# manyeyes/K2TransducerAsr

Measured on AMD Instinct MI355X. Metric: RTFx (audio-sec/wall-sec) offline Zipformer greedy, higher is better.
Workload: dtype f32

## Files before the change

include/k2hip_debug.h:

```cpp
#ifndef K2HIP_DEBUG_H
#define K2HIP_DEBUG_H
#include "k2hip.h"

#ifdef __cplusplus
extern "C" {
#endif
#if defined(__GNUC__)
#pragma GCC visibility push(default)
#endif


int32_t k2hip_debug_search_retries(k2hip_model_t* model, int32_t* n);
int32_t k2hip_debug_decoder_table_check(k2hip_model_t* model, int32_t n_samples, uint32_t seed, int64_t* rows, int64_t* mismatched);
int32_t k2hip_debug_beam_trace(k2hip_model_t* model, int32_t* trace, int64_t cap_words, int32_t* B, int32_t* Tprime, int32_t* beam);

int32_t k2hip_debug_stream_hotword_uploads(k2hip_model_t* model, int32_t* uploads, int32_t* resident);
int32_t k2hip_debug_beam_launch_counts(int64_t* plain, int64_t* hotwords);

int32_t k2hip_debug_poison_stream(k2hip_online_stream_t* s);
int32_t k2hip_debug_stream_mirrored(const k2hip_online_stream_t* s, int32_t* ok);

int32_t k2hip_debug_gemm_run(k2hip_model_t* model, const float* A, const float* W, const float* bias, const float* res, float* C,
                             int32_t M, int32_t N, int32_t K, int32_t act, int32_t glu, int32_t glu_cols, int32_t cfg);
int32_t k2hip_debug_op_run(k2hip_model_t* model, const char* op, const int64_t* iargs, int32_t n_iargs, void* const* bufs,
                           const int64_t* buf_bytes, int32_t n_bufs, uint32_t out_mask);

int32_t k2hip_debug_kws_stream_get_state(const k2hip_kws_stream_t* s, float* a, int32_t* start, int32_t cap);
int32_t k2hip_debug_keywords_get_tables(const k2hip_keywords_t* kw, int32_t* parent, int32_t* tok, int32_t* depth, int32_t* keyword, float* bar,
                                        int32_t cap);
int32_t k2hip_debug_kws_ref_dp(const int32_t* parent, const int32_t* depth, const int32_t* keyword, const float* bar, int32_t S, const float* stay,
                               const float* emit, int32_t T, float* a, int32_t* start, int32_t* ev_keyword, int32_t* ev_start, int32_t* ev_end,
                               float* ev_sum, int32_t cap, int32_t* n_events);

int32_t k2hip_debug_ctc_kws_stream_get_state(const k2hip_ctc_kws_stream_t* s, float* v, int32_t* st, int32_t cap);
int32_t k2hip_debug_ctc_kws_ref_dp(const int32_t* parent, const int32_t* tok, const int32_t* depth, const int32_t* keyword, const float* bar,
                                   const int32_t* rc, int32_t S, const float* log_probs, int32_t V, int32_t T, float* v, int32_t* st,
                                   int32_t* ev_keyword, int32_t* ev_start, int32_t* ev_end, float* ev_sum, int32_t cap, int32_t* n_events);

int32_t k2hip_debug_gemm(k2hip_model_t* model, int32_t M, int32_t N, int32_t K, int32_t act, int32_t with_res, int32_t cfg,
                         int32_t iters, float* ms);
int32_t k2hip_debug_gemm_check(k2hip_model_t* model, int32_t M, int32_t N, int32_t K, int32_t act, int32_t with_res, int32_t cfg,
                               int32_t iters, float* ms, float* max_err);
int32_t k2hip_debug_gemm_trace(k2hip_model_t* model, int32_t M, int32_t N, int32_t K, int32_t act, int32_t with_res, int32_t cfg,
                               unsigned long long* out, int64_t cap, int32_t* n_wg, int32_t* n_waves);

#if defined(__GNUC__)
#pragma GCC visibility pop
#endif
#ifdef __cplusplus
}
#endif
#endif
```

k2transducerasr_amd/csrc/api.cpp:

```cpp
#include <algorithm>
#include <atomic>
#include <cmath>
#include <fstream>
#include <iterator>
#include <map>
#include <memory>
#include <mutex>
#include <new>

#include "text.h"
#include "engine.h"
#include "beam_hist.h"
#include "ctc_prefix_hist.h"
#include "hotwords.h"
#include "keywords.h"
#include "kws_ref.h"
#include "ctc_kws_ref.h"
#include "ngram_lm.h"
#include "../../include/k2hip_debug.h"

using namespace k2hip;

struct PinVec {
    Engine* e = nullptr;
// ... 2484 lines not shown
int32_t k2hip_debug_decoder_table_check(k2hip_model_t* model, int32_t n_samples, uint32_t seed,
                                                                                int64_t* rows, int64_t* mismatched) {
    return guard([&] {
        NEED(model); NEED(rows); NEED(mismatched);
        K2_REQUIRE(n_samples >= 0 && n_samples <= 65536, "decoder table check: %d samples", n_samples);
        EngineLock lk(model->engine);
        long long r = 0, m = 0;
        model->engine.decoder_table_check(n_samples, seed, &r, &m);
        *rows = r;
        *mismatched = m;
    });
}
int32_t k2hip_debug_poison_stream(k2hip_online_stream_t* s) {
    return guard([&] {
        NEED(s);
        s->poisoned = true;
    });
}

int32_t k2hip_debug_stream_mirrored(const k2hip_online_stream_t* s, int32_t* ok) {
    return guard([&] {
        NEED(s); NEED(ok);
        *ok = s->mir_ok ? 1 : 0;
    });
}

int32_t k2hip_debug_set_switch(const char* env_name, int32_t value) {
    return guard([&] {
        NEED(env_name);
        tunables_init_from_env();
        if (!tunables_set(env_name, value)) failf(K2HIP_ERR_INVALID, "unknown switch '%s'", env_name);
    });
}
int32_t k2hip_debug_gemm(k2hip_model_t* model, int32_t M, int32_t N, int32_t K,
                                                                 int32_t act, int32_t with_res, int32_t cfg, int32_t iters, float* ms) {
    return guard([&] {
        NEED(model); NEED(ms);
        EngineLock lk(model->engine);
        *ms = model->engine.debug_gemm(M, N, K, act, with_res != 0, iters, cfg, nullptr);
    });
}
int32_t k2hip_debug_gemm_check(k2hip_model_t* model, int32_t M, int32_t N, int32_t K,
                                                                       int32_t act, int32_t with_res, int32_t cfg, int32_t iters, float* ms,
                                                                       float* max_err) {
    return guard([&] {
        NEED(model); NEED(ms); NEED(max_err);
        EngineLock lk(model->engine);
        *ms = model->engine.debug_gemm(M, N, K, act, with_res != 0, iters, cfg, max_err);
    });
}

int32_t k2hip_debug_gemm_run(k2hip_model_t* model, const float* A, const float* W, const float* bias, const float* res, float* C, int32_t M,
                             int32_t N, int32_t K, int32_t act, int32_t glu, int32_t glu_cols, int32_t cfg) {
    return guard([&] {
        NEED(model); NEED(A); NEED(W); NEED(C);
        EngineLock lk(model->engine);
        model->engine.debug_gemm_host(A, W, bias, res, C, M, N, K, act, glu, glu_cols, cfg);
    });
}

int32_t k2hip_debug_op_run(k2hip_model_t* model, const char* op, const int64_t* iargs, int32_t n_iargs, void* const* bufs,
                           const int64_t* buf_bytes, int32_t n_bufs, uint32_t out_mask) {
    return guard([&] {
        NEED(model); NEED(op);
        if (!Engine::debug_op) failf(K2HIP_ERR_UNSUPPORTED, "debug_op_run: this build has no kernels");
        EngineLock lk(model->engine);
// ... 245 lines not shown
```

k2transducerasr_amd/csrc/engine.cpp:

```cpp
#include <cstring>
#include <thread>

#include "engine.h"
#include "lattice_ref.h"
#include "ctc_lattice_ref.h"
#include "kws_ref.h"
#include "ctc_kws_ref.h"
#include "ctc_prefix_bias_ref.h"
#include "ctc_prefix_ref.h"
#include "hotwords.h"
#include "ngram_lm.h"

#include <climits>
#include <cmath>

namespace k2hip {

namespace {
constexpr int kTailFrames = 19;
}

Engine::Engine(const std::string& weights, const char* overrides, int device) : device_(device) {
    tunables_init_from_env();
    model_.reset(new Model(weights, overrides));
// ... 381 lines not shown
            std::swap(src, src_alt);
            return;
        }
        linear(c, src, D, wi, bi, hid, HV, M, D, HV);
        if (site) {
            attn_av_out_ring(c, aw, ring(k == 1 ? lay_.val1[gl] : lay_.val2[gl]), hid, wo, bo, src, B, T, KL, KLp, H, vh, D);
            return;
        }
        if (attn_av_out(c, aw, hid, wo, bo, src, B, T, T, KLp, H, vh, D)) return;
        GemmArgs g;
        g.A = aw; g.lda = KLp; g.sA0 = (long long)T * KLp; g.sA1 = (long long)B * T * KLp;
        g.W = hid; g.w_kn = 1; g.ldw = HV; g.sW0 = (long long)T * HV; g.sW1 = vh;
        g.C = tmp; g.ldc = HV; g.sC0 = (long long)T * HV; g.sC1 = vh;
        g.M = T; g.N = vh; g.K = T; g.nb0 = B; g.nb1 = H;
        gemm(c, g);
        linear(c, tmp, HV, wo, bo, src, D, M, HV, D, ACT_NONE, src, D);
    };
    auto conv_module = [&](int k) {
        if (site) {
            const long long cache_off = k == 1 ? lay_.conv1[gl] : lay_.conv2[gl];
            const float *wc = wk("conv_module%d.depthwise_conv.causal_conv.weight", k), *bc = wk("conv_module%d.depthwise_conv.causal_conv.bias", k);
            const float *ww = wk("conv_module%d.depthwise_conv.chunkwise_conv.weight", k), *bw = wk("conv_module%d.depthwise_conv.chunkwise_conv.bias", k);
            const float* sc = wk("conv_module%d.depthwise_conv.chunkwise_conv_scale", k);
            bool fused = false;
            if (!tunables().no_fused_conv)
                fused = gemm_glu_causal_conv(c, src, wk("conv_module%d.in_proj.weight#glu", k), wk("conv_module%d.in_proj.bias#glu", k), online_pool_, SS,
                                             cache_off, site->d_slots, wc, bc, ww, bw, sc, tmp2, B, T, D, K);
            if (!fused) {
                linear(c, src, D, wk("conv_module%d.in_proj.weight", k), wk("conv_module%d.in_proj.bias", k), hid, 2 * D, M, D, 2 * D);
                glu_causal_conv(c, hid, online_pool_, SS, cache_off, site->d_slots, wc, bc, ww, bw, sc, tmp2, B, T, D, K);
            }
        } else {
            const float *wd = wk("conv_module%d.depthwise_conv.weight#kd", k), *bd = wk("conv_module%d.depthwise_conv.bias", k);
            if (M >= 256 && !tunables().no_glu_epilogue) {
                GemmArgs g;
                g.A = src; g.lda = D; g.W = wk("conv_module%d.in_proj.weight#glu", k); g.ldw = D; g.bias = wk("conv_module%d.in_proj.bias#glu", k);
                g.C = hid; g.ldc = D; g.M = M; g.N = 2 * D; g.K = D; g.glu = 1;
                gemm(c, g);
                dwconv1d_swoosh(c, hid, wd, bd, tmp2, B, T, D, K);
            } else {
                linear(c, src, D, wk("conv_module%d.in_proj.weight", k), wk("conv_module%d.in_proj.bias", k), hid, 2 * D, M, D, 2 * D);
                glu_dwconv1d_swoosh(c, hid, wd, bd, tmp2, B, T, D, K);
            }
        }
        linear(c, tmp2, D, wk("conv_module%d.out_proj.weight", k), wk("conv_module%d.out_proj.bias", k), src, D, M, D, D, ACT_NONE, src, D);
    };

    linear(c, cat, ldcat, w("feed_forward1.out_proj.weight"), w("feed_forward1.out_proj.bias"), src, D, M, F1, D, ACT_NONE, x, D);
    nonlin_attention();
    self_attn(1);
    conv_module(1);
    {
        linear(c, src, D, w("feed_forward2.in_proj.weight"), w("feed_forward2.in_proj.bias"), hid, F, M, D, F, ACT_SWOOSH_L);
        GemmArgs g;
        g.A = hid; g.lda = F; g.W = w("feed_forward2.out_proj.weight"); g.ldw = F; g.bias = w("feed_forward2.out_proj.bias");
        g.C = src; g.ldc = D; g.M = M; g.N = D; g.K = F; g.res = src; g.ldr = D;
        g.byp_orig = x; g.ld_orig = D; g.byp_scale = w("bypass_mid.bypass_scale");
        gemm(c, g);
    }
    self_attn(2);
    conv_module(2);
    feed_forward(3, F * 5 / 4, src, src);
    if (tail && tail->bias2)
        biasnorm_bypass_downsample(c, src, x, w("norm.bias"), w("norm.log_scale"), w("bypass.bypass_scale"), x, tail->bias2, tail->xd2, B, T, D,
                                   tail->ds2, tail->D2);
    else
        biasnorm_bypass(c, src, x, w("norm.bias"), w("norm.log_scale"), w("bypass.bypass_scale"), x, M, D);
// ... 1781 lines not shown
            g.glu = I(); g.glu_cols = I();
            g.ldm = I(); g.sM0 = L(); g.sM1 = L();
            g.ld_orig = I();
            const int cfg = I(), res_is_C = I();
            const long long oA = L(), oW = L(), oR = L(), oC = L(), oM = L(), oO = L();
            float *A = P(), *W = P(), *bias = P(), *res = P(), *C = P();
            const int* skip = reinterpret_cast<const int*>(P());
            float *mul = P(), *orig = P(), *scale = P();
            int* plan_out = reinterpret_cast<int*>(P());
            K2_REQUIRE(A && W && C && plan_out && buf_bytes[n_bufs - 1] >= 20, "debug_op_run gemm: A, W, C and a plan buffer of 5 ints are needed");
            K2_REQUIRE(!(res_is_C && res), "debug_op_run gemm: res_is_C takes no res buffer");
            K2_REQUIRE(oA >= 0 && oW >= 0 && oR >= 0 && oC >= 0 && oM >= 0 && oO >= 0, "debug_op_run gemm: negative offset");
            if (res_is_C) res = C;
            g.A = A + oA; g.W = W + oW; g.bias = bias; g.res = res ? res + oR : nullptr; g.C = C + oC;
            g.skip_if_zero = skip;
            g.mul = mul ? mul + oM : nullptr;
            g.byp_orig = orig ? orig + oO : nullptr; g.byp_scale = scale;
            GemmForceGuard force(cfg);
            const GemmPlan pl = plan_gemm(g, gemm_force());
            const int rep[5] = {(int)pl.family, pl.idx, pl.BM, pl.BN, pl.mode};
            K2_HIP(copy_blocking(plan_out, rep, sizeof rep, hipMemcpyHostToDevice));
            gemm(c, g);
        } else if (name == "gemm_glu_causal_conv") {
            float *x = P(), *wg = P(), *bg = P(), *pool = P();
            const long long ss = L(), off = L();
            const int* slots = reinterpret_cast<const int*>(P());
            float *wc = P(), *bc = P(), *ww = P(), *bw = P(), *sc = P(), *y = P();
            const int B = I(), Tc = I(), D = I(), K = I();
            int* entry_out = reinterpret_cast<int*>(P());
            K2_REQUIRE(entry_out && buf_bytes[n_bufs - 1] >= 4, "debug_op_run gemm_glu_causal_conv: an entry buffer of 1 int is needed");
            const int entry = glu_conv_ring_entry(B, Tc, D, K);
            K2_HIP(copy_blocking(entry_out, &entry, sizeof entry, hipMemcpyHostToDevice));
            took = gemm_glu_causal_conv(c, x, wg, bg, pool, ss, off, slots, wc, bc, ww, bw, sc, y, B, Tc, D, K);
        } else if (name == "biasnorm") {
            float *x = P(), *bias = P(), *ls = P(), *y = P();
            const int M = I(), D = I();
            biasnorm(c, x, bias, ls, y, M, D);
        } else if (name == "bypass") {
            float *orig = P(), *x = P(), *scale = P(), *y = P();
            const int M = I(), D = I();
            bypass(c, orig, x, scale, y, M, D);
        } else if (name == "biasnorm_bypass") {
            float *x = P(), *orig = P(), *nb = P(), *ls = P(), *scale = P(), *y = P();
            const int M = I(), D = I();
            biasnorm_bypass(c, x, orig, nb, ls, scale, y, M, D);
        } else if (name == "biasnorm_bypass_downsample") {
            float *x = P(), *orig = P(), *nb = P(), *ls = P(), *scale = P(), *y = P(), *bias2 = P(), *xd2 = P();
            const int B = I(), T = I(), D = I(), ds2 = I(), D2 = I();
            biasnorm_bypass_downsample(c, x, orig, nb, ls, scale, y, bias2, xd2, B, T, D, ds2, D2);
        } else if (name == "downsample") {
            float *x = P(), *bias = P(), *y = P();
            const int B = I(), T = I(), D = I(), ds = I(), Din = I();
            downsample(c, x, bias, y, B, T, D, ds, Din);
        } else if (name == "downsample_full") {
            FullDimSegs s;
            s.n = I();
            K2_REQUIRE(s.n >= 1 && s.n <= 8, "debug_op_run downsample_full: %d segments", s.n);
            for (int k = 0; k < s.n; k++) s.ld[k] = I();
            for (int k = 0; k < s.n; k++) s.col1[k] = I();
            s.lz_Td = I(); s.lz_ds = I(); s.lz_Do = I();
            for (int k = 0; k < s.n; k++) s.src[k] = P();
            s.lz_orig = P(); s.lz_xd = P(); s.lz_scale = P();
            float *bias = P(), *y = P();
            const int B = I(), T = I(), D = I(), ds = I();
            downsample_full(c, s, bias, y, B, T, D, ds);
        } else if (name == "upsample_combine") {
// ... 764 lines not shown
```

k2transducerasr_amd/csrc/gemm.hip:

```cpp
#include <algorithm>
#include <cmath>
#include <cstdlib>
#include <map>
#include <mutex>
#include <type_traits>

#include "act.h"
#include "kernels.h"

#pragma clang diagnostic ignored "-Winline-asm"

namespace k2hip {

typedef float f32x16 __attribute__((ext_vector_type(16)));
typedef float f32x4 __attribute__((ext_vector_type(4)));

namespace {


__device__ __forceinline__ float apply_act(float v, int act) {
    switch (act) {
        case ACT_SWOOSH_L: return swoosh_l(v);
        case ACT_SWOOSH_R: return swoosh_r(v);
        case ACT_TANH: {
// ... 471 lines not shown
                if (e == 0 && gk < 3) {
                    __builtin_amdgcn_sched_barrier(0);
#pragma unroll
                    for (int i = 0; i < MT; i++)
                        fa[nx][i] = *reinterpret_cast<const float4*>(sa + i * 32 * BK + (((2 * (gk + 1) + lh) ^ swa) << 2));
#pragma unroll
                    for (int j = 0; j < NT; j++)
                        fb[nx][j] = *reinterpret_cast<const float4*>(sb + j * 32 * BK + (((2 * (gk + 1) + lh) ^ swb) << 2));
                    __builtin_amdgcn_sched_barrier(0);
                }
            }
        }
    }

    K2_DMA_STAMP()
#pragma unroll
    for (int j = 0; j < NT; j++)
#pragma unroll
        for (int i = 0; i < MT; i++) {
            float vals[16];
#pragma unroll
            for (int r = 0; r < 16; r++) vals[r] = acc[i][j][r];
            epilogue_rows<16, Rows32>(g, vals, m0 + wr * WM + i * 32 + 4 * lh, n0 + wc * WN + j * 32 + li, C, nullptr, rres[i][j], R != nullptr,
                                      nullptr, g.bias ? g.bias + z0 * g.sBias0 : nullptr);
        }
    K2_DMA_STAMP()
    if (stamp && lane == 0) {
        stamp[62] = nstamp;
        stamp[63] = __builtin_amdgcn_s_memrealtime();
    }
#undef K2_DMA_STAMP
}

template <int BM, int BN, int WM, int WN, int NST>
__global__ __launch_bounds__(64 * (BM / WM) * (BN / WN)) void gemm_f32_mfma_pipe(GemmArgs g) {
    constexpr int BK = 32;
    constexpr int MT = WM / 32, NT = WN / 32;
    constexpr int WCOLS = BN / WN;
    constexpr int NW = (BM / WM) * (BN / WN);
    constexpr int NINST = (BM + BN) / 8;
    constexpr int IPW = NINST / NW;
    constexpr int STAGE = (BM + BN) * BK;
    constexpr int DPE = (IPW + 3) / 4;
    static_assert(NST == 3 || NST == 4, "pipe: three or four stages");
    static_assert(NINST % NW == 0, "pipe: every wave issues the same number of DMA instructions");
    static_assert((NST - 2) * IPW <= 63 && MT <= 4 && NT <= 2, "pipe: counted wait / wave tile out of range");

    if (g.skip_if_zero && *g.skip_if_zero == 0) return;
    extern __shared__ __attribute__((aligned(16))) float smem[];

    const int tid = threadIdx.x;
    const int lane = tid & 63, wave = __builtin_amdgcn_readfirstlane(tid >> 6);
    const int wr = wave / WCOLS, wc = wave % WCOLS;
    const int li = lane & 31, lh = lane >> 5;
    float* __restrict__ C = g.C;
    const float* __restrict__ R = g.res;
    int mb_, nb_;
    xcd_tile(mb_, nb_, g.xcd_panels == 1 ? 0 : g.M, g.N);
    const int m0 = mb_ * BM, n0 = nb_ * BN;
    const int nk = g.K / BK;

    unsigned long long* stamp = g.dbg ? g.dbg + ((size_t)(blockIdx.x + blockIdx.y * gridDim.x) * NW + wave) * 64 : nullptr;
    int nstamp = 0;
#define K2_PIPE_STAMP()                                                    \
    if (stamp) {  \
        if (lane == 0) stamp[nstamp] = __builtin_amdgcn_s_memtime();       \
        nstamp++;                                                          \
    }
    if (stamp && lane == 0) stamp[60] = __builtin_amdgcn_s_memrealtime();
    K2_PIPE_STAMP()

    const unsigned lds_base = (unsigned)(unsigned long long)(__attribute__((address_space(3))) char*)smem;
    unsigned voff[IPW];
    unsigned long long sb[IPW];
    unsigned mq[IPW];
#pragma unroll
    for (int q = 0; q < IPW; q++) {
        const int inst = wave + q * NW;
        const int slot = inst * 64 + lane;
        const int r = slot >> 3, cp = slot & 7;
        const int c = cp ^ ((r >> 1) & 7);
        const bool is_a = inst < BM / 8;
        const long long row = is_a ? min(m0 + r, g.M - 1) : min(n0 + (r - BM), g.N - 1);
        voff[q] = (unsigned)((row * (is_a ? g.lda : g.ldw) + 4 * c) * 4);
        const unsigned long long base = (unsigned long long)(is_a ? g.A : g.W);
        sb[q] = ((unsigned long long)(unsigned)__builtin_amdgcn_readfirstlane((int)(base >> 32)) << 32) |
                (unsigned long long)(unsigned)__builtin_amdgcn_readfirstlane((int)(unsigned)base);
        mq[q] = __builtin_amdgcn_readfirstlane(lds_base + inst * 1024);
    }

#define K2_PIPE_DMA(ST_, KT_, q_)                                                                                          \
    {                                                                                                                      \
// ... 66 lines not shown
        }

    f32x16 acc[MT][NT];
#pragma unroll
    for (int i = 0; i < MT; i++)
#pragma unroll
        for (int j = 0; j < NT; j++)
#pragma unroll
            for (int r = 0; r < 16; r++) acc[i][j][r] = 0.f;
    f32x4 fa[2][MT], fb[2][NT];
    K2_PIPE_STAMP()
    if (nk >= NST - 1) asm volatile("s_waitcnt vmcnt(%0)" ::"n"((NST - 2) * IPW) : "memory");
    else asm volatile("s_waitcnt vmcnt(0)" ::: "memory");
    __builtin_amdgcn_s_barrier();
    K2_PIPE_READ(0, 0, 0)
    K2_PIPE_STAMP()
    float rres[MT][NT][16];
    if (R) {
#pragma unroll
        for (int j = 0; j < NT; j++) {
            const int col = min(n0 + wc * WN + j * 32 + li, g.N - 1);
#pragma unroll
            for (int i = 0; i < MT; i++)
#pragma unroll
                for (int r = 0; r < 16; r++) {
                    const int row = min(m0 + wr * WM + i * 32 + (r & 3) + 8 * (r >> 2) + 4 * lh, g.M - 1);
                    rres[i][j][r] = R[(long long)row * g.ldr + col];
                }
        }
    }
    float bias_pre[NT];
#pragma unroll
    for (int j = 0; j < NT; j++) bias_pre[j] = g.bias ? g.bias[min(n0 + wc * WN + j * 32 + li, g.N - 1)] : 0.f;

    int kt = 0;
    const int nsteady = nk - (NST - 1);
    for (; kt + NST <= nsteady; kt += NST) {
        K2_PIPE_STEP(0, kt, true, true, K2_PIPE_WAIT_STEADY)
        K2_PIPE_STEP(1, kt + 1, true, true, K2_PIPE_WAIT_STEADY)
        K2_PIPE_STEP(2, kt + 2, true, true, K2_PIPE_WAIT_STEADY)
        if (NST == 4) { K2_PIPE_STEP(NST == 4 ? 3 : 0, kt + 3, true, true, K2_PIPE_WAIT_STEADY) }
    }
#define K2_PIPE_S(j_) K2_PIPE_STEP((j_) % NST, kt + (j_), true, true, K2_PIPE_WAIT_STEADY)
#define K2_PIPE_T(j_) K2_PIPE_STEP((j_) % NST, kt + (j_), true, false, K2_PIPE_WAIT_DRAIN)
#define K2_PIPE_L(j_) K2_PIPE_STEP((j_) % NST, kt + (j_), false, false, K2_PIPE_WAIT_DRAIN)
    const int rs = nsteady - kt;
    if (NST == 3) {
        switch (rs) {
            case 0: K2_PIPE_T(0) K2_PIPE_L(1) break;
            case 1: K2_PIPE_S(0) K2_PIPE_T(1) K2_PIPE_L(2) break;
            default: K2_PIPE_S(0) K2_PIPE_S(1) K2_PIPE_T(2) K2_PIPE_L(3) break;
        }
    } else {
        switch (rs) {
            case 0: K2_PIPE_T(0) K2_PIPE_T(1) K2_PIPE_L(2) break;
            case 1: K2_PIPE_S(0) K2_PIPE_T(1) K2_PIPE_T(2) K2_PIPE_L(3) break;
            case 2: K2_PIPE_S(0) K2_PIPE_S(1) K2_PIPE_T(2) K2_PIPE_T(3) K2_PIPE_L(4) break;
            default: K2_PIPE_S(0) K2_PIPE_S(1) K2_PIPE_S(2) K2_PIPE_T(3) K2_PIPE_T(4) K2_PIPE_L(5) break;
        }
    }
#undef K2_PIPE_S
#undef K2_PIPE_T
#undef K2_PIPE_L
    K2_PIPE_STAMP()
#undef K2_PIPE_WAIT_DRAIN
#undef K2_PIPE_WAIT_STEADY
#undef K2_PIPE_STEP
#undef K2_PIPE_FRAGS_READY
#undef K2_PIPE_READ
#undef K2_PIPE_DMA

#pragma unroll
    for (int j = 0; j < NT; j++)
#pragma unroll
        for (int i = 0; i < MT; i++) {
            float vals[16];
#pragma unroll
            for (int r = 0; r < 16; r++) vals[r] = acc[i][j][r];
            epilogue_rows<16, Rows32>(g, vals, m0 + wr * WM + i * 32 + 4 * lh, n0 + wc * WN + j * 32 + li, C, nullptr, rres[i][j], R != nullptr,
                                      nullptr, g.bias, true, bias_pre[j]);
        }
    K2_PIPE_STAMP()
    if (stamp && lane == 0) {
        stamp[62] = nstamp;
        stamp[63] = __builtin_amdgcn_s_memrealtime();
    }
#undef K2_PIPE_STAMP
}

template <int BM, int BN, int WM, int WN, int NST>
__global__ __launch_bounds__(64 * (BM / WM) * (BN / WN)) void gemm_f32_mfma_p16(GemmArgs g) {
    constexpr int BK = 32;
    constexpr int MT = WM / 16, NT = WN / 16;
    constexpr int WCOLS = BN / WN;
    constexpr int NW = (BM / WM) * (BN / WN);
    constexpr int NINST = (BM + BN) / 8;
    constexpr int IPW = NINST / NW;
    constexpr int STAGE = (BM + BN) * BK;
    constexpr int DPE = (IPW + 3) / 4;
    static_assert(NST == 3, "p16: three stages");
    static_assert(NINST % NW == 0, "p16: every wave issues the same number of DMA instructions");
    static_assert(MT >= 1 && NT >= 1 && MT * NT <= 12, "p16: wave tile");

    if (g.skip_if_zero && *g.skip_if_zero == 0) return;
// ... 644 lines not shown
    lds_attr.ensure(gemm_f32_mfma_dma<BM, BN, WM, WN, NST>, (int)lds);
    hipLaunchKernelGGL((gemm_f32_mfma_dma<BM, BN, WM, WN, NST>), grid, dim3(64 * (BM / WM) * (BN / WN)), lds, ctx.stream, a);
}

template <int BM, int BN, int KS, int NST, int LW, int PF = 0>
void launch_ring(const Ctx& ctx, const GemmArgs& a) {
    dim3 grid(cdiv(a.N, BN), cdiv(a.M, BM), a.nb0 * a.nb1);
    size_t lds = sizeof(float) * std::max((size_t)NST * KS * (BM + BN) * 32, KS > 1 ? (size_t)KS * (BM / 32) * (BN / 32) * 1024 : (size_t)0) + (PF ? 256 : 0);
    static LdsAttrOnce lds_attr;
    lds_attr.ensure(gemm_f32_mfma_ring<BM, BN, KS, NST, LW, PF>, (int)lds);
    hipLaunchKernelGGL((gemm_f32_mfma_ring<BM, BN, KS, NST, LW, PF>), grid, dim3(64 * ((BM / 32) * (BN / 32) * KS + LW + PF)), lds, ctx.stream, a);
}

template <int BM, int BN, int KS, int NST, int PF = 0>
void launch_ring_conv(const Ctx& ctx, const GemmArgs& a) {
    dim3 grid(cdiv(a.N, BN), cdiv(a.M, BM), 1);
    const int pad = a.cf_K >> 1, Kc = (a.cf_K + 1) >> 1, CH = BN / 2;
    const size_t conv_fl = (size_t)(BM / a.cf_Tc) * CH * (pad + a.cf_Tc) + (size_t)CH * (Kc | 1) + (size_t)CH * a.cf_K;
    size_t lds = sizeof(float) * std::max({(size_t)NST * KS * (BM + BN) * 32, KS > 1 ? (size_t)KS * (BM / 32) * (BN / 32) * 1024 : (size_t)0, conv_fl}) + (PF ? 256 : 0);
    static LdsAttrOnce lds_attr;
    lds_attr.ensure(gemm_f32_mfma_ring<BM, BN, KS, NST, 0, PF, true>, (int)lds);
    hipLaunchKernelGGL((gemm_f32_mfma_ring<BM, BN, KS, NST, 0, PF, true>), grid, dim3(64 * ((BM / 32) * (BN / 32) * KS + PF)), lds, ctx.stream, a);
}

template <int BM, int BN, int WM, int WN, int NST>
void launch_pipe(const Ctx& ctx, const GemmArgs& a) {
    dim3 grid(cdiv(a.N, BN), cdiv(a.M, BM), 1);
    size_t lds = sizeof(float) * NST * (BM + BN) * 32;
    static LdsAttrOnce lds_attr;
    lds_attr.ensure(gemm_f32_mfma_pipe<BM, BN, WM, WN, NST>, (int)lds);
    K2_REQUIRE((long long)a.M * a.lda < (1ll << 29) && (long long)a.N * a.ldw < (1ll << 29), "pipe: operand too large for 31-bit lane byte offsets");
    K2_REQUIRE(a.K % 32 == 0 && a.K >= 32 * (NST - 1), "pipe: K %d too short for %d stages", a.K, NST);
    hipLaunchKernelGGL((gemm_f32_mfma_pipe<BM, BN, WM, WN, NST>), grid, dim3(64 * (BM / WM) * (BN / WN)), lds, ctx.stream, a);
}

template <int BM, int BN, int WM, int WN, int NST>
void launch_p16(const Ctx& ctx, const GemmArgs& a) {
    dim3 grid(cdiv(a.N, BN), cdiv(a.M, BM), 1);
    size_t lds = sizeof(float) * NST * (BM + BN) * 32;
    static LdsAttrOnce lds_attr;
    lds_attr.ensure(gemm_f32_mfma_p16<BM, BN, WM, WN, NST>, (int)lds);
    K2_REQUIRE((long long)a.M * a.lda < (1ll << 29) && (long long)a.N * a.ldw < (1ll << 29), "p16: operand too large for 31-bit lane byte offsets");
    K2_REQUIRE(a.K % 32 == 0 && a.K >= 32 * (NST - 1) && !a.glu, "p16: K %d too short for %d stages, or a gated epilogue", a.K, NST);
    hipLaunchKernelGGL((gemm_f32_mfma_p16<BM, BN, WM, WN, NST>), grid, dim3(64 * (BM / WM) * (BN / WN)), lds, ctx.stream, a);
}

template <int BM, int BN, int WM, int WN, int BK, int MODE>
void launch_cfg(const Ctx& ctx, const GemmArgs& a) {
    constexpr int LDSK = BK + 4;
    dim3 grid(cdiv(a.N, BN), cdiv(a.M, BM), a.nb0 * a.nb1);
    size_t lds = sizeof(float) * 2 * (BM + BN) * LDSK;
    static LdsAttrOnce lds_attr;
    lds_attr.ensure(gemm_f32_mfma<BM, BN, WM, WN, BK, MODE>, (int)lds);
    hipLaunchKernelGGL((gemm_f32_mfma<BM, BN, WM, WN, BK, MODE>), grid, dim3(64 * (BM / WM) * (BN / WN)), lds, ctx.stream, a);
}

template <int MODE>
void launch_reg(const Ctx& ctx, const GemmArgs& a, int idx) {
    switch (idx) {
#define X(i, bm, bn, wm, wn, bk) case i: launch_cfg<bm, bn, wm, wn, bk, MODE>(ctx, a); break;
        K2_REG_TABLE(X)
#undef X
    }
}

template <int E>
// ... 72 lines not shown
    K2_HIP(hipGetLastError());
    if (ctx.instrument && ctx.gemm_log)
        ctx.gemm_log->push_back({a.M, a.N, a.K, a.nb0 * a.nb1, a.act, a.res != nullptr, gemm_kind(a, p), 0.f});
    if (ctx.instrument) K2_HIP(hipEventRecord(ctx.next_event(), ctx.stream));
}

bool gemm_glu_causal_conv(const Ctx& ctx, const float* x, const float* wg, const float* bg, float* pool, long long slot_stride, long long off,
                          const int* slots, const float* wc, const float* bc, const float* ww, const float* bw, const float* sc, float* y, int B,
                          int Tc, int D, int K) {
    const int M = B * Tc, N = 2 * D;
    const int entry = glu_conv_ring_entry(B, Tc, D, K);
    if (entry < 0) return false;
    const double fl = 2.0 * M * (double)N * D;
    ctx.add_flops(fl, 2.0 * M * (double)D * (K + (K + 1) / 2), 1);
    if (ctx.dry) return true;
    GemmArgs g;
    g.A = x; g.lda = D; g.W = wg; g.ldw = D; g.bias = bg; g.C = y; g.ldc = D; g.M = M; g.N = N; g.K = D;
    g.cf_pool = pool; g.cf_stride = slot_stride; g.cf_off = off; g.cf_slots = slots;
    g.cf_wc = wc; g.cf_bc = bc; g.cf_ww = ww; g.cf_bw = bw; g.cf_sc = sc; g.cf_Tc = Tc; g.cf_K = K;
    g.xcd_panels = tunables().xcd_panels;
    if (ctx.instrument) K2_HIP(hipEventRecord(ctx.next_event(), ctx.stream));
    if (ctx.instrument && ctx.gemm_log) ctx.gemm_log->push_back({M, N, D, 1, 0, 0, 64, 0.f});
    switch (entry) {
        case 16: launch_ring_conv_entry<16>(ctx, g); break;
        case 17: launch_ring_conv_entry<17>(ctx, g); break;
        case 12: launch_ring_conv_entry<12>(ctx, g); break;
        default: launch_ring_conv_entry<8>(ctx, g); break;
    }
    K2_HIP(hipGetLastError());
    if (ctx.instrument) K2_HIP(hipEventRecord(ctx.next_event(), ctx.stream));
    return true;
}

void linear(const Ctx& ctx, const float* A, int lda, const float* W, const float* bias, float* C, int ldc, int M, int K,
            int N, int act, const float* res, int ldr) {
    GemmArgs g;
    g.A = A; g.lda = lda; g.W = W; g.ldw = K; g.bias = bias; g.C = C; g.ldc = ldc;
    g.M = M; g.N = N; g.K = K; g.act = act; g.res = res; g.ldr = ldr;
    gemm(ctx, g);
}

}
```

k2transducerasr_amd/csrc/gemm_plan.cpp:

```cpp
#include "kernels.h"

namespace k2hip {

namespace {

GemmForce g_force;

bool entry(GemmFamily f, int idx, GemmPlan* p) {
    p->family = f;
    p->idx = idx;
    switch (f) {
#define X(i, bm, bn, wm, wn, bk_or_nst) case i: p->BM = bm; p->BN = bn; p->waves = (bm / wm) * (bn / wn); return true;
        case GemmFamily::REG: switch (idx) { K2_REG_TABLE(X) } return false;
        case GemmFamily::DMA: switch (idx) { K2_DMA_TABLE(X) } return false;
        case GemmFamily::PIPE: switch (idx) { K2_PIPE_TABLE(X) } return false;
        case GemmFamily::P16: switch (idx) { K2_P16_TABLE(X) } return false;
#undef X
        case GemmFamily::RING: {
            if (idx < 0 || idx >= (int)(sizeof(kRing) / sizeof(kRing[0]))) return false;
            const RingCfg& r = kRing[idx];
            p->BM = r.BM;
            p->BN = r.BN;
            p->waves = (r.BM / 32) * (r.BN / 32) * r.KS + r.LW + r.PF;
            return true;
// ... 130 lines not shown
            if (tiles >= 128 && cost < best_cost) return make(GemmFamily::P16, 0, f.ablate);
        }
        return make(GemmFamily::PIPE, best, f.ablate);
    }
    if (dma_ok && (cfg == 5 || cfg == 0 || (cfg >= 7 && cfg <= 11))) return make(GemmFamily::DMA, cfg == 7 ? 5 : cfg, f.ablate);
    GemmPlan r = make(GemmFamily::REG, cfg == 7 || cfg == 8 || cfg == 11 ? 5 : (cfg <= 5 || cfg == 12) ? cfg : 2, f.ablate);
    r.mode = a.cv_Fout > 0 ? MODE_CONV : a.w_kn ? MODE_WKN : MODE_PLAIN;
    return r;
}

int gemm_kind(const GemmArgs& a, const GemmPlan& p) {
    const int base = a.cv_Fout > 0 ? 1 : (a.w_kn ? 2 : 0);
    switch (p.family) {
        case GemmFamily::REG: return base;
        case GemmFamily::DMA: return base + 16;
        case GemmFamily::SKINNY3: case GemmFamily::SKINNY6: case GemmFamily::SKINNY6_8: return base + 32;
        case GemmFamily::RING: return base + 64;
        case GemmFamily::PIPE: return base + 128 + 256 * (p.BM / 32) + 4096 * (p.BN / 32);
        case GemmFamily::P16: return base + 128 + 256 * (p.BM / 32) + 4096 * (p.BN / 32) + (1 << 20);
    }
    return base;
}

int glu_conv_ring_entry(int B, int Tc, int D, int K) {
    const int M = B * Tc, N = 2 * D;
    if (Tc < 2 || 32 % Tc != 0 || D % 64 != 0 || (K != 31 && K != 15 && K != 7)) return -1;
    int e = small_ring_entry(M, N, D);
    if (e < 0) e = 8;
    const RingCfg& r = kRing[e];
    if ((long long)(r.BM / Tc) * (r.BN / 2) * (K >> 1) > 8ll * (r.BM / 32) * (r.BN / 32) * r.KS * 64) return -1;
    return e;
}

}
```

k2transducerasr_amd/csrc/kernels.h:

```cpp
#pragma once
#include "ctc_prefix_layout.h"
#include "common.h"

namespace k2hip {

#ifdef K2HIP_DEV
#define K2HIP_DEV_SWITCH(name, def) int name = def
#else
#define K2HIP_DEV_SWITCH(name, def) static constexpr int name = def
#endif
struct Tunables {
    int no_glu_epilogue = 0;
    int attn_long = 0;
    int no_fused_av = 0;
    int fused_vproj_min_t = 4;
    int no_fused_vproj = 0;
    int no_fused_conv = 0;
    int conformer_gemm_scores = 0;
    int dw7_tiled = 0;
    int dw1d_tt = 0;
    int lstm_seq = 0;
    int greedy_one_part = 0;
    int greedy_parts = 0;
    int beam_launches = 0;
// ... 63 lines not shown
    const float* W = nullptr;
    const float* bias = nullptr;
    const float* res = nullptr;
    float* C = nullptr;
    int M = 0, N = 0, K = 0;
    int lda = 0, ldw = 0, ldc = 0, ldr = 0;
    int act = ACT_NONE;
    int xcd_panels = 0;
    int act_cols = 0;
    int w_kn = 0;
    int nb0 = 1, nb1 = 1;
    const int* skip_if_zero = nullptr;
    long long sA0 = 0, sA1 = 0, sW0 = 0, sW1 = 0, sC0 = 0, sC1 = 0, sR0 = 0, sR1 = 0;
    long long sBias0 = 0;
    int cv_Fout = 0, cv_Tout = 0, cv_Tin = 0, cv_Fin = 0, cv_C = 0, cv_st = 1, cv_sf = 1;
    int seg_len = 0, seg_stride = 0;
    int res_div = 1;
    int act_after_res = 0;
    int glu = 0;
    int glu_cols = 0;
    const float* mul = nullptr;
    int ldm = 0;
    long long sM0 = 0, sM1 = 0;
    const float* byp_orig = nullptr;
    const float* byp_scale = nullptr;
    int ld_orig = 0;
    float* cf_pool = nullptr;
    long long cf_stride = 0, cf_off = 0;
    const int* cf_slots = nullptr;
    const float *cf_wc = nullptr, *cf_bc = nullptr, *cf_ww = nullptr, *cf_bw = nullptr, *cf_sc = nullptr;
    int cf_Tc = 0, cf_K = 0;
    unsigned long long* dbg = nullptr;
    int ablate = 0;
};
void gemm(const Ctx& ctx, const GemmArgs& a);
bool gemm_glu_causal_conv(const Ctx& ctx, const float* x, const float* wg, const float* bg, float* pool, long long slot_stride, long long off,
                          const int* slots, const float* wc, const float* bc, const float* ww, const float* bw, const float* sc, float* y, int B,
                          int Tc, int D, int K);

#define K2_PIPE_TABLE(X)                                                                                                       \
    X(0, 128, 64, 64, 32, 3) X(1, 128, 64, 32, 32, 3) X(2, 128, 128, 64, 64, 3) X(3, 128, 128, 64, 32, 3) X(4, 128, 64, 64, 32, 4)  \
    X(5, 64, 64, 32, 32, 3) X(6, 128, 128, 64, 64, 4) X(7, 64, 128, 32, 64, 3) X(8, 128, 128, 32, 32, 3) X(9, 128, 64, 32, 32, 4) \
    X(10, 64, 64, 64, 32, 3) X(11, 64, 64, 32, 64, 3) X(12, 256, 64, 64, 32, 3) X(13, 128, 32, 32, 32, 3) X(14, 128, 32, 64, 32, 3)
#define K2_P16_TABLE(X) X(0, 64, 96, 32, 48, 3) X(1, 128, 96, 64, 48, 3) X(2, 64, 192, 32, 96, 3) X(3, 32, 96, 16, 48, 3)
#define K2_RING_TABLE(X)                                                                                        \
    X(0, 128, 64, 1, 2, 0, 0) X(1, 128, 64, 1, 3, 0, 0) X(2, 128, 64, 1, 2, 0, 1) X(3, 128, 64, 1, 3, 0, 1) X(4, 128, 64, 1, 4, 0, 1)   \
    X(5, 64, 64, 1, 3, 0, 0) X(6, 64, 64, 1, 3, 0, 1) X(7, 64, 64, 1, 4, 0, 1) X(8, 64, 64, 2, 3, 0, 0) X(9, 64, 64, 2, 3, 0, 1)      \
    X(10, 64, 64, 4, 2, 0, 0) X(11, 64, 64, 4, 2, 0, 1) X(12, 32, 64, 2, 3, 0, 0) X(13, 32, 64, 4, 3, 0, 0) X(14, 32, 64, 4, 3, 0, 1)  \
    X(15, 32, 32, 4, 3, 0, 0) X(16, 32, 32, 4, 4, 0, 1) X(17, 64, 32, 4, 3, 0, 0) X(18, 128, 128, 1, 2, 0, 0) X(19, 128, 128, 1, 2, 0, 1) \
    X(20, 64, 128, 1, 3, 0, 0) X(21, 64, 128, 1, 3, 0, 1) X(22, 64, 96, 1, 3, 0, 0) X(23, 64, 96, 1, 3, 0, 1) X(24, 128, 96, 1, 2, 0, 1) \
    X(25, 128, 64, 1, 3, 2, 0) X(26, 128, 64, 1, 3, 2, 1) X(27, 128, 64, 2, 2, 0, 1) X(28, 64, 96, 2, 3, 0, 0) X(29, 64, 96, 2, 2, 0, 0) \
    X(30, 64, 96, 2, 2, 0, 1) X(31, 128, 96, 1, 3, 0, 0) X(32, 128, 96, 1, 3, 0, 1)
struct RingCfg { int BM, BN, KS, NST, LW, PF; };
#define X(i, bm, bn, ks, nst, lw, pf) {bm, bn, ks, nst, lw, pf},
constexpr RingCfg kRing[] = {K2_RING_TABLE(X)};
#undef X
#define K2_DMA_TABLE(X)                                                                                                          \
    X(0, 128, 128, 64, 32, 3) X(5, 128, 64, 32, 32, 2) X(8, 128, 64, 32, 32, 4) X(9, 64, 64, 32, 32, 2) X(10, 64, 64, 32, 32, 3) \
    X(11, 64, 96, 32, 32, 2) X(20, 32, 32, 32, 32, 4) X(21, 32, 64, 32, 32, 4)
#define K2_REG_TABLE(X)                                                                                                           \
    X(0, 128, 128, 64, 32, 32) X(1, 128, 128, 64, 32, 64) X(2, 64, 64, 32, 32, 32) X(3, 64, 64, 32, 32, 64) X(4, 128, 64, 32, 32, 64) \
    X(5, 128, 64, 32, 32, 32) X(12, 128, 32, 32, 32, 32)
enum GemmMode { MODE_PLAIN = 0, MODE_CONV = 1, MODE_WKN = 2 };

enum class GemmFamily { REG, DMA, PIPE, P16, RING, SKINNY3, SKINNY6, SKINNY6_8 };
struct GemmPlan {
    GemmFamily family = GemmFamily::REG;
    int idx = 0;
    int mode = MODE_PLAIN;
    int ablate = 0;
    int BM = 0, BN = 0, waves = 0;
};
struct GemmForce {
    enum Kind { AUTO, CFG, RING, PIPE, P16 } kind = AUTO;
    int idx = -1;
    int ablate = 0;
    bool dma = true;
};
GemmForce decode_gemm_force(int code);
GemmPlan plan_gemm(const GemmArgs& a, const GemmForce& f);
int gemm_kind(const GemmArgs& a, const GemmPlan& p);
int glu_conv_ring_entry(int B, int Tc, int D, int K);
void debug_force_gemm_cfg(int code);
GemmForce gemm_force();
struct GemmForceGuard {
    explicit GemmForceGuard(int code) { debug_force_gemm_cfg(code); }
    ~GemmForceGuard() { debug_force_gemm_cfg(-1); }
    GemmForceGuard(const GemmForceGuard&) = delete;
    GemmForceGuard& operator=(const GemmForceGuard&) = delete;
};
void linear(const Ctx& ctx, const float* A, int lda, const float* W, const float* bias, float* C, int ldc, int M, int K,
            int N, int act = ACT_NONE, const float* res = nullptr, int ldr = 0);

struct RingRef {
    float* pool = nullptr;
    long long slot_stride = 0;
    long long off = 0;
    const int* slots = nullptr;
    const int* chunks = nullptr;
};

void attn_scores_softmax(const Ctx& ctx, const float* qkp, int ld, const float* pp, float* aw, int B, int T, int Tp, int H, int qh = 32,
                         int koff0 = -1, int poff0 = -1);

bool attn_av_out(const Ctx& ctx, const float* aw, const float* v, const float* wout, const float* bias, float* x, int B, int T, int KL, int Tp,
                 int H, int vh, int D);
bool attn_av_out_ring(const Ctx& ctx, const float* aw, const RingRef& vals, const float* newrows, const float* wout, const float* bias, float* x,
                      int B, int T, int KL, int Tp, int H, int vh, int D);
void attn_proj_av_out_ring(const Ctx& ctx, const float* aw, const RingRef& vals, const float* xin, const float* win, const float* bin,
                           const float* wout, const float* bias, float* xout, int B, int T, int KL, int Tp, int H, int vh, int D);

void nonlin_av_out_ring(const Ctx& ctx, const float* aw, const RingRef& cache, const float* hid, int ldh, const float* wout, const float* bias,
                        float* x, int B, int T, int KL, int Tp, int Hc, int D);

void pad_logfloor(const Ctx& ctx, const float* packed, const long long* d_off, const long long* d_len, float* out, int B,
// ... 437 lines not shown
```

Before: 23890.

## Fuse offline conv-module GLU GEMM with depthwise conv and SwooshR epilogue

For the offline (non-streaming) Zipformer conv module, the pipe MFMA GEMM gains a templated epilogue. It applies bias and GLU, stages the gated rows of a whole stream in LDS with zero padding, runs the depthwise 1D conv (K=15 or 31) and SwooshR, then writes the final output. This removes the intermediate hidden tensor's global write and read and a separate conv kernel launch. It only applies when a whole stream fits in one row tile (T <= BM), and the planner rejects cases where one-tile-per-stream would add waves. Otherwise it falls back to the old path.

New measurement: 24170, median of 6. 1.2% higher.

```diff
diff --git a/include/k2hip_debug.h b/include/k2hip_debug.h
--- a/include/k2hip_debug.h
+++ b/include/k2hip_debug.h
@@ -22,6 +22,7 @@
 
 int32_t k2hip_debug_gemm_run(k2hip_model_t* model, const float* A, const float* W, const float* bias, const float* res, float* C,
                              int32_t M, int32_t N, int32_t K, int32_t act, int32_t glu, int32_t glu_cols, int32_t cfg);
+int32_t k2hip_debug_conv_fused_plan(int32_t B, int32_t T, int32_t D, int32_t K, int32_t streaming, int32_t* entry);
 int32_t k2hip_debug_op_run(k2hip_model_t* model, const char* op, const int64_t* iargs, int32_t n_iargs, void* const* bufs,
                            const int64_t* buf_bytes, int32_t n_bufs, uint32_t out_mask);
 
diff --git a/k2transducerasr_amd/csrc/api.cpp b/k2transducerasr_amd/csrc/api.cpp
--- a/k2transducerasr_amd/csrc/api.cpp
+++ b/k2transducerasr_amd/csrc/api.cpp
@@ -2540,6 +2540,13 @@
         if (!tunables_set(env_name, value)) failf(K2HIP_ERR_INVALID, "unknown switch '%s'", env_name);
     });
 }
+int32_t k2hip_debug_conv_fused_plan(int32_t B, int32_t T, int32_t D, int32_t K, int32_t streaming, int32_t* entry) {
+    return guard([&] {
+        NEED(entry);
+        tunables_init_from_env();
+        *entry = glu_dwconv_pipe_entry(B, T, D, K, streaming != 0);
+    });
+}
 int32_t k2hip_debug_gemm(k2hip_model_t* model, int32_t M, int32_t N, int32_t K,
                                                                  int32_t act, int32_t with_res, int32_t cfg, int32_t iters, float* ms) {
     return guard([&] {
diff --git a/k2transducerasr_amd/csrc/engine.cpp b/k2transducerasr_amd/csrc/engine.cpp
--- a/k2transducerasr_amd/csrc/engine.cpp
+++ b/k2transducerasr_amd/csrc/engine.cpp
@@ -437,7 +437,9 @@
             }
         } else {
             const float *wd = wk("conv_module%d.depthwise_conv.weight#kd", k), *bd = wk("conv_module%d.depthwise_conv.bias", k);
-            if (M >= 256 && !tunables().no_glu_epilogue) {
+            const bool fused = gemm_glu_dwconv1d(c, src, wk("conv_module%d.in_proj.weight#glu", k), wk("conv_module%d.in_proj.bias#glu", k), wd, bd, tmp2, B, T, D, K);
+            if (fused) {
+            } else if (M >= 256 && !tunables().no_glu_epilogue) {
                 GemmArgs g;
                 g.A = src; g.lda = D; g.W = wk("conv_module%d.in_proj.weight#glu", k); g.ldw = D; g.bias = wk("conv_module%d.in_proj.bias#glu", k);
                 g.C = hid; g.ldc = D; g.M = M; g.N = 2 * D; g.K = D; g.glu = 1;
@@ -2285,6 +2287,47 @@
             const int entry = glu_conv_ring_entry(B, Tc, D, K);
             K2_HIP(copy_blocking(entry_out, &entry, sizeof entry, hipMemcpyHostToDevice));
             took = gemm_glu_causal_conv(c, x, wg, bg, pool, ss, off, slots, wc, bc, ww, bw, sc, y, B, Tc, D, K);
+        } else if (name == "gemm_glu_dwconv1d") {
+            const int wg_k = nbuf + 1, bg_k = nbuf + 2;
+            float *x = P(), *wg = P(), *bg = P(), *wd = P(), *bd = P(), *y = P();
+            const int B = I(), T = I(), D = I(), K = I();
+            int* entry_out = reinterpret_cast<int*>(P());
+            K2_REQUIRE(x && wg && bg && wd && bd && y && entry_out && buf_bytes[n_bufs - 1] >= 4, "debug_op_run gemm_glu_dwconv1d: six operands and an entry buffer of 1 int are needed");
+            K2_REQUIRE(B >= 1 && T >= 1 && D >= 16 && D % 16 == 0 && K >= 1, "debug_op_run gemm_glu_dwconv1d: B %d T %d D %d K %d", B, T, D, K);
+            const int M = B * T;
+            const int entry = glu_dwconv_pipe_entry(B, T, D, K, false);
+            K2_HIP(copy_blocking(entry_out, &entry, sizeof entry, hipMemcpyHostToDevice));
+            auto scratch = [&](size_t floats) {
+                char* p = nullptr;
+                K2_HIP(hipMalloc(&p, floats * sizeof(float)));
+                d.base.push_back(p);
+                return reinterpret_cast<float*>(p);
+            };
+            const bool fused = gemm_glu_dwconv1d(c, x, wg, bg, wd, bd, y, B, T, D, K);
+            if (fused) {
+            } else if (M >= 256 && !tunables().no_glu_epilogue) {
+                float* hid = scratch((size_t)M * D);
+                GemmArgs g;
+                g.A = x; g.lda = D; g.W = wg; g.ldw = D; g.bias = bg;
+                g.C = hid; g.ldc = D; g.M = M; g.N = 2 * D; g.K = D; g.glu = 1;
+                gemm(c, g);
+                dwconv1d_swoosh(c, hid, wd, bd, y, B, T, D, K);
+            } else {
+                const float *hw = static_cast<const float*>(bufs[wg_k]), *hb = static_cast<const float*>(bufs[bg_k]);
+                std::vector<float> vw((size_t)2 * D * D), vb((size_t)2 * D);
+                for (int ch = 0; ch < D; ch++) {
+                    const int rv = 32 * (ch / 16) + ch % 16, rg = rv + 16;
+                    memcpy(&vw[(size_t)ch * D], &hw[(size_t)rv * D], sizeof(float) * D);
+                    memcpy(&vw[(size_t)(D + ch) * D], &hw[(size_t)rg * D], sizeof(float) * D);
+                    vb[ch] = hb[rv];
+                    vb[D + ch] = hb[rg];
+                }
+                float *wp = scratch(vw.size()), *bp = scratch(vb.size()), *hid = scratch((size_t)M * 2 * D);
+                K2_HIP(copy_blocking(wp, vw.data(), vw.size() * sizeof(float), hipMemcpyHostToDevice));
+                K2_HIP(copy_blocking(bp, vb.data(), vb.size() * sizeof(float), hipMemcpyHostToDevice));
+                linear(c, x, D, wp, bp, hid, 2 * D, M, D, 2 * D);
+                glu_dwconv1d_swoosh(c, hid, wd, bd, y, B, T, D, K);
+            }
         } else if (name == "biasnorm") {
             float *x = P(), *bias = P(), *ls = P(), *y = P();
             const int M = I(), D = I();
diff --git a/k2transducerasr_amd/csrc/gemm.hip b/k2transducerasr_amd/csrc/gemm.hip
--- a/k2transducerasr_amd/csrc/gemm.hip
+++ b/k2transducerasr_amd/csrc/gemm.hip
@@ -527,7 +527,7 @@
 #undef K2_DMA_STAMP
 }
 
-template <int BM, int BN, int WM, int WN, int NST>
+template <int BM, int BN, int WM, int WN, int NST, int DWK = 0>
 __global__ __launch_bounds__(64 * (BM / WM) * (BN / WN)) void gemm_f32_mfma_pipe(GemmArgs g) {
     constexpr int BK = 32;
     constexpr int MT = WM / 32, NT = WN / 32;
@@ -552,7 +552,7 @@
     const float* __restrict__ R = g.res;
     int mb_, nb_;
     xcd_tile(mb_, nb_, g.xcd_panels == 1 ? 0 : g.M, g.N);
-    const int m0 = mb_ * BM, n0 = nb_ * BN;
+    const int m0 = DWK > 0 ? mb_ * g.dw_T : mb_ * BM, n0 = nb_ * BN;
     const int nk = g.K / BK;
 
     unsigned long long* stamp = g.dbg ? g.dbg + ((size_t)(blockIdx.x + blockIdx.y * gridDim.x) * NW + wave) * 64 : nullptr;
@@ -685,6 +685,15 @@
     float bias_pre[NT];
 #pragma unroll
     for (int j = 0; j < NT; j++) bias_pre[j] = g.bias ? g.bias[min(n0 + wc * WN + j * 32 + li, g.N - 1)] : 0.f;
+    constexpr int DW_CH = BN / 2, DW_TT = DWK > 0 ? BM * DW_CH / (64 * NW) : 1;
+    static_assert(DWK == 0 || (DW_TT == 8 && DWK % 2 == 1 && (BM + DWK - 1) * DW_CH <= NST * STAGE), "pipe: conv tail's tile form");
+    float dw_tap[DWK > 0 ? DWK : 1], dw_bias = 0.f;
+    if constexpr (DWK > 0) {
+        const float* wp = g.dw_w + (n0 >> 1) + (tid & (DW_CH - 1));
+        dw_bias = g.dw_b[(n0 >> 1) + (tid & (DW_CH - 1))];
+#pragma unroll
+        for (int q = 0; q < DWK; q++) dw_tap[q] = wp[(long long)q * (g.N >> 1)];
+    }
 
     int kt = 0;
     const int nsteady = nk - (NST - 1);
@@ -723,6 +732,56 @@
 #undef K2_PIPE_READ
 #undef K2_PIPE_DMA
 
+    if constexpr (DWK > 0) {
+        constexpr int HALF = DWK / 2, lgCH = DW_CH == 64 ? 6 : DW_CH == 32 ? 5 : 4;
+        static_assert(DW_CH == 1 << lgCH, "pipe: conv tail's channel count");
+        const int T = g.dw_T;
+        float* xs = smem;
+        __syncthreads();
+        for (int e = tid; e < 2 * HALF * DW_CH; e += 64 * NW) {
+            const int r = e >> lgCH;
+            xs[((r < HALF ? r : T + r) << lgCH) + (e & (DW_CH - 1))] = 0.f;
+        }
+#pragma unroll
+        for (int j = 0; j < NT; j++)
+#pragma unroll
+            for (int i = 0; i < MT; i++) {
+                const int ch = ((wc * WN + j * 32) >> 1) + (li & 15), lrow0 = wr * WM + i * 32 + 4 * lh;
+#pragma unroll
+                for (int r = 0; r < 16; r++) {
+                    const float v = acc[i][j][r] + bias_pre[j];
+                    const float other = __shfl_xor(v, 16, 64);
+                    const float gated = v * (1.0f / (1.0f + __expf(-other)));
+                    const int lrow = lrow0 + Rows32::off(r);
+                    if ((li & 16) == 0 && lrow < T) xs[((HALF + lrow) << lgCH) + ch] = gated;
+                }
+            }
+        __syncthreads();
+        const int ch = tid & (DW_CH - 1), t0 = (tid >> lgCH) * DW_TT;
+        if (t0 < T) {
+            float o[DW_TT];
+#pragma unroll
+            for (int i = 0; i < DW_TT; i++) o[i] = dw_bias;
+            const float* xp = xs + (t0 << lgCH) + ch;
+#pragma unroll
+            for (int r = 0; r < DW_TT + DWK - 1; r++) {
+                const float xv = xp[r << lgCH];
+#pragma unroll
+                for (int i = 0; i < DW_TT; i++)
+                    if (r - i >= 0 && r - i < DWK) o[i] = __builtin_fmaf(dw_tap[r - i], xv, o[i]);
+            }
+            float* yp = C + (long long)(m0 + t0) * g.ldc + (n0 >> 1) + ch;
+#pragma unroll
+            for (int i = 0; i < DW_TT; i++)
+                if (t0 + i < T) yp[(long long)i * g.ldc] = swoosh_r(o[i]);
+        }
+        K2_PIPE_STAMP()
+        if (stamp && lane == 0) {
+            stamp[62] = nstamp;
+            stamp[63] = __builtin_amdgcn_s_memrealtime();
+        }
+        return;
+    }
 #pragma unroll
     for (int j = 0; j < NT; j++)
 #pragma unroll
@@ -1433,6 +1492,27 @@
     K2_REQUIRE((long long)a.M * a.lda < (1ll << 29) && (long long)a.N * a.ldw < (1ll << 29), "pipe: operand too large for 31-bit lane byte offsets");
     K2_REQUIRE(a.K % 32 == 0 && a.K >= 32 * (NST - 1), "pipe: K %d too short for %d stages", a.K, NST);
     hipLaunchKernelGGL((gemm_f32_mfma_pipe<BM, BN, WM, WN, NST>), grid, dim3(64 * (BM / WM) * (BN / WN)), lds, ctx.stream, a);
+}
+
+template <int BM, int BN, int WM, int WN, int NST, int DWK>
+void launch_pipe_dwconv(const Ctx& ctx, const GemmArgs& a) {
+    dim3 grid(a.N / BN, a.M / a.dw_T, 1);
+    size_t lds = sizeof(float) * NST * (BM + BN) * 32;
+    static LdsAttrOnce lds_attr;
+    lds_attr.ensure(gemm_f32_mfma_pipe<BM, BN, WM, WN, NST, DWK>, (int)lds);
+    K2_REQUIRE((long long)a.M * a.lda < (1ll << 29) && (long long)a.N * a.ldw < (1ll << 29), "pipe: operand too large for 31-bit lane byte offsets");
+    K2_REQUIRE(a.K % 32 == 0 && a.K >= 32 * (NST - 1), "pipe: K %d too short for %d stages", a.K, NST);
+    K2_REQUIRE(a.dw_K == DWK && a.dw_T >= 1 && a.dw_T <= BM && a.M % a.dw_T == 0 && a.N % BN == 0 && a.ldc >= a.N / 2 && a.dw_w && a.dw_b,
+               "pipe: conv tail needs whole streams of <= %d frames and whole column tiles (T %d, M %d, N %d)", BM, a.dw_T, a.M, a.N);
+    hipLaunchKernelGGL((gemm_f32_mfma_pipe<BM, BN, WM, WN, NST, DWK>), grid, dim3(64 * (BM / WM) * (BN / WN)), lds, ctx.stream, a);
+}
+template <int DWK>
+void launch_pipe_dwconv_entry(const Ctx& ctx, const GemmArgs& a, int idx) {
+    switch (idx) {
+        case 1: launch_pipe_dwconv<128, 64, 32, 32, 3, DWK>(ctx, a); break;
+        case 5: launch_pipe_dwconv<64, 64, 32, 32, 3, DWK>(ctx, a); break;
+        default: launch_pipe_dwconv<128, 128, 32, 32, 3, DWK>(ctx, a); break;
+    }
 }
 
 template <int BM, int BN, int WM, int WN, int NST>
@@ -1571,6 +1651,32 @@
     return true;
 }
 
+bool gemm_glu_dwconv1d(const Ctx& ctx, const float* x, const float* wg, const float* bg, const float* wd, const float* bd, float* y, int B, int T,
+                       int D, int K) {
+    const int M = B * T, N = 2 * D;
+    const int entry = glu_dwconv_pipe_entry(B, T, D, K, false);
+    if (entry < 0) return false;
+    ctx.add_flops(2.0 * M * (double)N * D, 2.0 * M * (double)D * K, 1);
+    if (ctx.dry) return true;
+    GemmArgs g;
+    g.A = x; g.lda = D; g.W = wg; g.ldw = D; g.bias = bg; g.C = y; g.ldc = D; g.M = M; g.N = N; g.K = D;
+    g.dw_w = wd; g.dw_b = bd; g.dw_K = K; g.dw_T = T;
+    g.xcd_panels = tunables().xcd_panels;
+    if (ctx.instrument) K2_HIP(hipEventRecord(ctx.next_event(), ctx.stream));
+    if (ctx.instrument && ctx.gemm_log) {
+        GemmPlan p;
+        p.family = GemmFamily::PIPE;
+        p.BM = entry == 5 ? 64 : 128;
+        p.BN = entry == 8 ? 128 : 64;
+        ctx.gemm_log->push_back({M, N, D, 1, 0, 0, gemm_kind(g, p), 0.f});
+    }
+    if (K == 15) launch_pipe_dwconv_entry<15>(ctx, g, entry);
+    else launch_pipe_dwconv_entry<31>(ctx, g, entry);
+    K2_HIP(hipGetLastError());
+    if (ctx.instrument) K2_HIP(hipEventRecord(ctx.next_event(), ctx.stream));
+    return true;
+}
+
 void linear(const Ctx& ctx, const float* A, int lda, const float* W, const float* bias, float* C, int ldc, int M, int K,
             int N, int act, const float* res, int ldr) {
     GemmArgs g;
diff --git a/k2transducerasr_amd/csrc/gemm_plan.cpp b/k2transducerasr_amd/csrc/gemm_plan.cpp
--- a/k2transducerasr_amd/csrc/gemm_plan.cpp
+++ b/k2transducerasr_amd/csrc/gemm_plan.cpp
@@ -186,4 +186,22 @@
     return e;
 }
 
-}
+int glu_dwconv_pipe_entry(int B, int T, int D, int K, bool streaming) {
+    if (streaming || tunables().no_fused_conv || tunables().no_glu_epilogue) return -1;
+    if (B < 1 || T < 1 || D < 1) return -1;
+    const long long M = (long long)B * T;
+    if (M < 256 || M * D >= (1ll << 29)) return -1;
+    if (K != 15 && K != 31) return -1;
+    if (gemm_force().kind != GemmForce::AUTO) return -1;
+    GemmArgs a;
+    a.M = (int)M; a.N = 2 * D; a.K = D; a.lda = D; a.ldw = D; a.ldc = D; a.glu = 1;
+    if (a.N <= 96 || a.N % 32 != 0) return -1;
+    const GemmPlan p = plan_gemm(a, GemmForce());
+    if (p.family != GemmFamily::PIPE || (p.idx != 1 && p.idx != 5 && p.idx != 8)) return -1;
+    if (T > p.BM || a.N % p.BN != 0) return -1;
+    const long long cols = a.N / p.BN;
+    if (cdiv((long long)B * cols, 256ll) > cdiv((long long)cdiv(M, (long long)p.BM) * cols, 256ll)) return -1;
+    return p.idx;
+}
+
+}
diff --git a/k2transducerasr_amd/csrc/kernels.h b/k2transducerasr_amd/csrc/kernels.h
--- a/k2transducerasr_amd/csrc/kernels.h
+++ b/k2transducerasr_amd/csrc/kernels.h
@@ -119,11 +119,17 @@
     int cf_Tc = 0, cf_K = 0;
     unsigned long long* dbg = nullptr;
     int ablate = 0;
+    const float* dw_w = nullptr;
+    const float* dw_b = nullptr;
+    int dw_K = 0, dw_T = 0;
 };
 void gemm(const Ctx& ctx, const GemmArgs& a);
 bool gemm_glu_causal_conv(const Ctx& ctx, const float* x, const float* wg, const float* bg, float* pool, long long slot_stride, long long off,
                           const int* slots, const float* wc, const float* bc, const float* ww, const float* bw, const float* sc, float* y, int B,
                           int Tc, int D, int K);
+
+bool gemm_glu_dwconv1d(const Ctx& ctx, const float* x, const float* wg, const float* bg, const float* wd, const float* bd, float* y, int B, int T,
+                       int D, int K);
 
 #define K2_PIPE_TABLE(X)                                                                                                       \
     X(0, 128, 64, 64, 32, 3) X(1, 128, 64, 32, 32, 3) X(2, 128, 128, 64, 64, 3) X(3, 128, 128, 64, 32, 3) X(4, 128, 64, 64, 32, 4)  \
@@ -168,6 +174,7 @@
 GemmPlan plan_gemm(const GemmArgs& a, const GemmForce& f);
 int gemm_kind(const GemmArgs& a, const GemmPlan& p);
 int glu_conv_ring_entry(int B, int Tc, int D, int K);
+int glu_dwconv_pipe_entry(int B, int T, int D, int K, bool streaming);
 void debug_force_gemm_cfg(int code);
 GemmForce gemm_force();
 struct GemmForceGuard {
```
